# askerlee/segtran

Hardware: AMD Instinct MI355X
Metric: train-step images/sec (cfg2, re-associated op order) (higher is better)
Workload: dtype f32; 1 GPU; REFUGE fundus 2D, segtran eff-b4, translayers 3, layercompress 1,1,2,2, 512x512, bs 6/GPU; global_batch=6, per_gpu_batch=6, parallelism=dp1, step=fwd+BCE/Dice+bwd+allreduce+clip+BertAdam, op_order=re-associated, ranks=1

## Files before the change

include/segx.h:

```cpp
#ifndef SEGX_H
#define SEGX_H
#include <stdint.h>
#ifdef __cplusplus
extern "C" {
#endif

int segx_version(void);
int segx_last_error(char* buf, int buflen);

enum { SEGX_EPI_NONE = 0, SEGX_EPI_GELU = 1 ,
       SEGX_EPI_SWISH = 2 ,
       SEGX_EPI_RELU = 3  };
enum { SEGX_BIAS_NONE = 0, SEGX_BIAS_N = 1 , SEGX_BIAS_M = 2  };
enum { SEGX_ENGINE_F32 = 0, SEGX_ENGINE_BF16X6 = 1 };
enum { SEGX_ENGINE_SEL_DEFAULT = 0, SEGX_ENGINE_SEL_F32 = 1, SEGX_ENGINE_SEL_BF16X6 = 2 };
enum { SEGX_TILE_AUTO = 0, SEGX_TILE_128x128 = 1, SEGX_TILE_64x64 = 2, SEGX_TILE_128x32 = 3, SEGX_TILE_32x128 = 4, SEGX_TILE_64x128 = 5,
       SEGX_TILE_256x128 = 6, SEGX_TILE_WS128x128 = 7, SEGX_TILE_WS128x256 = 8, SEGX_TILE_WS64x256 = 9,
       SEGX_TILE_WS96x256 = 10, SEGX_TILE_WS256x96 = 11,
       SEGX_TILE_SKINNY_NT = 12   };
typedef struct {
    int32_t M, N, K, nb0, nb1;
    int64_t a_b0, a_b1, a_m, a_k;
    int64_t b_b0, b_b1, b_n, b_k;
    int64_t c_b0, c_b1, c_m;
    float alpha;
    int32_t epilogue, bias_mode;
    int64_t bias_b1;
    const float* bias;
    float* aux;
    float* gmax;
    float dropout_p;
    uint64_t seed, offset;
    int32_t splitk;
    float* workspace;
    int32_t tile;
    int64_t bias_b0;
    int32_t batch_reduce;
    int32_t engine;
    const void* b_planes;
    int64_t bp_b0, bp_b1;
    const float* resid;
} segx_gemm_desc;
int segx_gemm_f32(const float* A, const float* B, float* C, const segx_gemm_desc* d, void* stream);
int segx_gemm_plan(const float* A, const float* B, const segx_gemm_desc* d, int* tile, int* splitk);
int segx_gemm_plan_model(const float* A, const float* B, const segx_gemm_desc* d, int* tile, int* splitk);
int segx_gemm_route(const float* A, const float* B, const segx_gemm_desc* d, int32_t* out);
int64_t segx_x6_presplit_elems(int rows, int K, int nb0, int nb1);
int segx_x6_presplit(const float* W, int rows, int K, int64_t s_row, int64_t s_k, int nb0, int nb1, int64_t s_b0, int64_t s_b1, void* planes, void* stream);


int segx_softmax_fwd(const float* S, float* P, float* Pdrop, int64_t rows, int L, float clip, const float* gmax,
                     float p, uint64_t seed, uint64_t offset, void* stream);
int segx_softmax_bwd(const float* P, const float* dPdrop, const float* S , float* dS,
                     int64_t rows, int L, float clip, const float* gmax, float p, uint64_t seed, uint64_t offset, void* stream);
int segx_posbias_fwd(const float* S, float* out, const float* table, int64_t nmat, int N, const int* geom, float weight, float clip,
                     const float* gmax, void* stream);
int segx_posbias_bwd(const float* dOut, const float* S, float* dS, float* dtable, int64_t nmat, int N, const int* geom, float weight,
                     float clip, void* stream);
int segx_layernorm_fwd(const float* X, const float* w, const float* b, float* Y, float* mean, float* rstd,
                       int64_t rows, int C, float eps, void* stream);
int segx_layernorm_bwd(const float* dY, const float* X, const float* w, const float* mean, const float* rstd, float* dX,
                       int64_t rows, int C, void* stream);
int64_t segx_colreduce_ws_floats(int64_t rows, int64_t C, int nout);
int segx_colsum(const float* X, float* out, float* ws, int64_t rows, int64_t C, void* stream);
int segx_ln_param_grad(const float* dY, const float* X, const float* mean, const float* rstd, float* dw, float* db,
                       float* ws, int64_t rows, int C, void* stream);
int segx_sum(const float* x, int64_t n, float* out, float* ws , float scale, void* stream);
int segx_rowsum(const float* X, float* out, int64_t R, int64_t S, void* stream);
int segx_prenorm_fwd(const float* X, const float* w1, const float* b1, const float* pos, int64_t pos_ld, float pos_weight,
                     const float* mask, float* Y, float* stats, int64_t B, int N, int C, float eps,
                     float p, uint64_t seed, uint64_t offset, void* stream);
int segx_prenorm_bwd(const float* dY, const float* X, const float* w1, const float* b1, const float* pos, int64_t pos_ld,
                     float pos_weight, const float* mask, const float* stats, float* dX, float* dU, int64_t B, int N, int C,
                     float p, uint64_t seed, uint64_t offset, void* stream);
int64_t segx_prenorm_bwd_all_ws_floats(int N, int C);
int segx_prenorm_bwd_all(const float* dY, const float* X, const float* w1, const float* b1, const float* pos, int64_t pos_ld, float pos_weight,
                         const float* mask, const float* stats, float* dX, float* dsum, float* dw, float* db, float* ws, int B, int N, int C,
                         float p, uint64_t seed, uint64_t offset, void* stream);
int segx_posembed_fwd(const float* posn, const float* Wp, const float* bp, float* out, float* stats, int64_t N, int C, int pd,
                      float eps, void* stream);
int segx_posembed_bwd(const float* dOut, const float* posn, const float* Wp, const float* bp, const float* stats, float* dZ,
                      int64_t N, int C, int pd, void* stream);
int segx_modes_aggr_fwd(const float* Z, const float* lnw, const float* lnb, const float* wa, const float* ba, float* Y, float* stats,
                        int Mo, int64_t R, int F, float eps, float p, uint64_t seed, uint64_t offset, void* stream);
int segx_modes_aggr_bwd(const float* dY, const float* Z, const float* lnw, const float* lnb, const float* wa, const float* stats,
                        float* dZ, float* dscore, int Mo, int64_t R, int F, float p, uint64_t seed, uint64_t offset, void* stream);
int segx_modes_aggr_param_grad(const float* dY, const float* Z, const float* lnw, const float* lnb, const float* wa,
                               const float* stats, const float* dscore, float* dlnw, float* dlnb, float* dwa, float* ws,
                               int Mo, int64_t R, int F, float p, uint64_t seed, uint64_t offset, void* stream);
int64_t segx_modes_aggr_bwd_all_ws_floats(int Mo, int64_t R, int F);
int segx_modes_aggr_bwd_all(const float* dY, const float* Z, const float* lnw, const float* lnb, const float* wa, const float* stats,
                            float* dZ, float* dscore, float* dlnw, float* dlnb, float* dwa, float* ws, int Mo, int64_t R, int F,
                            float p, uint64_t seed, uint64_t offset, void* stream);
int segx_gelu_bwd(const float* dH, const float* T, float* dT, int64_t n, float p, uint64_t seed, uint64_t offset, void* stream);
int64_t segx_gelu_bwd_colsum_ws_floats(int64_t rows, int N);
int segx_gelu_bwd_colsum(const float* dH, const float* T, float* dT, float* colsum, float* ws, int64_t rows, int N, float p, uint64_t seed, uint64_t offset,
                         void* stream);

int64_t segx_loss_ws_floats(int B, int C);
int segx_seg_loss_fwd(const float* logits, const float* mask, const float* pos_weight, const float* class_w, float* out,
                      float* ws, int B, int C, int64_t S, float dice_w, void* stream);
// ... 221 lines not shown
```

segtran_amd/csrc/gemm.hip:

```cpp
#include "gemm_x6ws.h"
#include "gemm_skinny.h"
#include "gemm_tuned.h"

namespace segx {

template <class Cfg, bool AKC, bool BKC, bool VEC, int EPI>
__global__ __launch_bounds__(256, 2) void gemm_f32_kernel(GemmArgs g) {
    __shared__ __attribute__((aligned(16))) TileLdsT<Cfg> lds;
    const TileCoord t = tile_coord<Cfg>(g);
    const DenseLoader<AKC, VEC, Cfg::BM> la{g.A + t.z0 * g.a_b0 + t.z1 * g.a_b1, g.a_m, g.a_k, t.m0, g.M};
    const DenseLoader<BKC, VEC, Cfg::BN> lb{g.B + t.z0 * g.b_b0 + t.z1 * g.b_b1, g.b_n, g.b_k, t.n0, g.N};
    f32x16 acc[Cfg::MI][Cfg::NJ];
    gemm_mainloop<Cfg>(acc, la, lb, t.kbeg, t.kend, lds);
    gemm_epilogue<EPI, Cfg>(acc, g, t);
}

template <class Cfg, bool AKC, bool BKC, int EPI, int WPE, int VAR = 0, int TERMS = 6>
__global__ __launch_bounds__(256) SEGX_MIN_WAVES_PER_SIMD(WPE) void gemm_x6_kernel(GemmArgs g) {
    __shared__ __attribute__((aligned(16))) unsigned char lds[X6Lds<Cfg, TERMS>::BYTES];
    const TileCoord t = tile_coord<Cfg>(g);
    const DenseLoader6<AKC, Cfg::BM> la{g.A + t.z0 * g.a_b0 + t.z1 * g.a_b1, g.a_m, g.a_k, t.m0, g.M};
    const DenseLoader6<BKC, Cfg::BN> lb{g.B + t.z0 * g.b_b0 + t.z1 * g.b_b1, g.b_n, g.b_k, t.n0, g.N};
    f32x16 acc[Cfg::MI][Cfg::NJ];
    gemm_mainloop_x6<Cfg, DenseLoader6<AKC, Cfg::BM>, DenseLoader6<BKC, Cfg::BN>, VAR, TERMS>(acc, la, lb, t.kbeg, t.kend, lds);
// ... 370 lines not shown
static GemmLaunch ws3_kernel(const GemmRoute& r) {
    switch (r.tile) {
        case SEGX_TILE_256x128: return ws3_tile<Cfg256x128>(r);
        case SEGX_TILE_WS128x128: return ws3_tile<Cfg128>(r);
        case SEGX_TILE_WS128x256: return ws3_tile<Cfg128x256>(r);
        case SEGX_TILE_WS64x256: return built_for<Cfg64x256>(gemm_x6ws_kernel<Cfg64x256, true, false, SEGX_EPI_NONE, 0, 3>);
        case SEGX_TILE_WS96x256: return ws3_tile<Cfg96x256>(r);
        default: return built_for<Cfg256x96>(gemm_x6ws_kernel<Cfg256x96, true, true, SEGX_EPI_NONE, 0, 3>);
    }
}
template <class Cfg> static GemmLaunch ws_pre_tile(const GemmRoute& r) {
    return built_for<Cfg>(by_flag(r.akc, [](auto ak) -> GemmKernel { return gemm_x6ws_pre_kernel<Cfg, decltype(ak)::value>; }));
}
static GemmLaunch route_kernel(const GemmRoute& r) {
    if (r.terms == 3) {
        switch (r.family) {
            case GEMM_X6: return x3_kernel<false>(r);
#ifndef SEGX_NO_LEAN
            case GEMM_X6_LEAN: return x3_kernel<true>(r);
#endif
            default: return ws3_kernel(r);
        }
    }
    switch (r.family) {
        case GEMM_X6: return r.sched ? x6_sched_kernel(r.sched) : x6_kernel<false>(r);
#ifndef SEGX_NO_LEAN
        case GEMM_X6_LEAN: return x6_kernel<true>(r);
#endif
        case GEMM_WS: return ws_kernel(r);
        case GEMM_WS_PRE: return r.tile == SEGX_TILE_256x128 ? ws_pre_tile<Cfg256x128>(r) : ws_pre_tile<Cfg128x256>(r);
        default: return f32_kernel(r);
    }
}
static void set_tiles(GemmArgs& g, const GemmLaunch& k, const GemmRoute& r) {
    g.tiles_m = ceil_div(g.M, k.bm); g.tiles_n = ceil_div(g.N, k.bn); g.mfast = r.walk ? tile_walk(g.M, g.N, g.K, g.tiles_m) : 0;
}
static int persistent_grid(const GemmArgs& g, const GemmRoute& r, int* grid) {
    const int64_t items = (int64_t)g.tiles_m * g.tiles_n * g.nbatch * g.splitk;
    SEGX_REQUIRE(items < 2147483647LL - 512, "segx_gemm_f32: too many tiles");
    *grid = (int)i64min(r.ws_grid, (items + 7) / 8 * 8);
    return 0;
}
static void slab_reduce(const segx_gemm_desc* d, float* C, const float* bias, int nslabs, bool skinny, hipStream_t stream) {
    const int64_t total = (int64_t)d->M * d->N;
    const float* ws = static_cast<const float*>(d->workspace);
    if (total * 16 <= 512 * 1024 && nslabs >= 16)
        hipLaunchKernelGGL((slab_sum_parts_kernel<16>), dim3((unsigned)((total + 15) / 16)), dim3(256), 0, stream, ws, C, bias, d->M, d->N, nslabs, total, d->c_m, d->alpha, d->bias_mode);
    else if (skinny || (total * 4 <= 1024 * 1024 && nslabs >= 4))
        hipLaunchKernelGGL((slab_sum_parts_kernel<4>), dim3((unsigned)((total + 63) / 64)), dim3(256), 0, stream, ws, C, bias, d->M, d->N, nslabs, total, d->c_m, d->alpha, d->bias_mode);
    else
        SEGX_SPLITK_REDUCE((unsigned)i64min(2048, (total + 255) / 256), stream, ws, C, bias, d->M, d->N, 1, nslabs, total, (int64_t)0, (int64_t)0, d->c_m, d->alpha,
                           d->bias_mode, (int64_t)0, (int64_t)0, total, (const float*)nullptr);
}
}

extern "C" int segx_gemm_plan(const float* A, const float* B, const segx_gemm_desc* d, int* tile, int* splitk) { return segx::gemm_plan_impl(A, B, d, tile, splitk, true); }
extern "C" int segx_gemm_plan_model(const float* A, const float* B, const segx_gemm_desc* d, int* tile, int* splitk) { return segx::gemm_plan_impl(A, B, d, tile, splitk, false); }

extern "C" int segx_gemm_route(const float* A, const float* B, const segx_gemm_desc* d, int32_t* out) {
    using namespace segx;
    SEGX_REQUIRE(A && B && d && out && d->M > 0 && d->N > 0 && d->K > 0 && d->nb0 > 0 && d->nb1 > 0, "segx_gemm_route: bad args");
    SEGX_REQUIRE(d->tile >= SEGX_TILE_AUTO && d->tile <= SEGX_TILE_SKINNY_NT && d->engine >= SEGX_ENGINE_SEL_DEFAULT && d->engine <= SEGX_ENGINE_SEL_BF16X6,
                 "segx_gemm_route: bad tile %d or engine selector %d", d->tile, d->engine);
    GemmRoute r;
    const int rc = gemm_route(A, B, d, &r);
    if (rc) return rc;
    out[0] = r.family; out[1] = r.tile; out[2] = r.terms; out[3] = r.splitk;
    return 0;
}

extern "C" int segx_gemm_f32(const float* A, const float* B, float* C, const segx_gemm_desc* d, void* stream_) {
    using namespace segx;
    hipStream_t stream = (hipStream_t)stream_;
    SEGX_REQUIRE(A && B && C && d, "segx_gemm_f32: null pointer");
    SEGX_REQUIRE(d->M > 0 && d->N > 0 && d->K > 0 && d->nb0 > 0 && d->nb1 > 0, "segx_gemm_f32: bad sizes M=%d N=%d K=%d nb=%dx%d",
                 d->M, d->N, d->K, d->nb0, d->nb1);
    SEGX_REQUIRE(d->a_m == 1 || d->a_k == 1, "segx_gemm_f32: A needs a unit stride (a_m=%lld a_k=%lld)", (long long)d->a_m, (long long)d->a_k);
    SEGX_REQUIRE(d->b_n == 1 || d->b_k == 1, "segx_gemm_f32: B needs a unit stride (b_n=%lld b_k=%lld)", (long long)d->b_n, (long long)d->b_k);
    SEGX_REQUIRE(d->epilogue == SEGX_EPI_NONE || d->epilogue == SEGX_EPI_GELU || d->epilogue == SEGX_EPI_SWISH || d->epilogue == SEGX_EPI_RELU, "segx_gemm_f32: bad epilogue %d", d->epilogue);
    SEGX_REQUIRE(d->epilogue != SEGX_EPI_RELU || (d->a_k == 1 && d->b_n == 1 && d->b_k != 1 && !d->resid && !d->gmax && d->dropout_p == 0.f),
                 "segx_gemm_f32: the relu epilogue is built for a pointwise convolution's forward (A k-contiguous, B row-contiguous; no resid, gmax or dropout)");
    SEGX_REQUIRE(d->epilogue != SEGX_EPI_SWISH || (d->a_k == 1 && d->b_n == 1 && d->b_k != 1 && !d->resid && !d->gmax && d->dropout_p == 0.f),
                 "segx_gemm_f32: the swish epilogue is built for a pointwise convolution's forward (A k-contiguous, B row-contiguous; no resid, gmax or dropout)");
    SEGX_REQUIRE(d->epilogue != SEGX_EPI_GELU || d->aux, "segx_gemm_f32: GELU epilogue needs aux");
    SEGX_REQUIRE(d->bias_mode == SEGX_BIAS_NONE || d->bias, "segx_gemm_f32: bias_mode set but bias null");
    SEGX_REQUIRE(d->dropout_p >= 0.f && d->dropout_p < 1.f, "segx_gemm_f32: dropout_p out of range");
    const int splitk = d->splitk > 1 ? d->splitk : 1;
    SEGX_REQUIRE(splitk == 1 || (d->workspace && d->epilogue == SEGX_EPI_NONE && !d->gmax), "segx_gemm_f32: split-K needs workspace and a plain epilogue");
    const bool breduce = d->batch_reduce != 0;
    SEGX_REQUIRE(!breduce || (d->workspace && d->epilogue == SEGX_EPI_NONE && !d->gmax), "segx_gemm_f32: batch_reduce needs workspace and a plain epilogue");
    SEGX_REQUIRE(!d->resid || (d->epilogue == SEGX_EPI_NONE && !breduce && !d->gmax), "segx_gemm_f32: resid needs a plain epilogue (no GELU, no batch_reduce, no gmax)");
    SEGX_REQUIRE(d->tile >= SEGX_TILE_AUTO && d->tile <= SEGX_TILE_SKINNY_NT, "segx_gemm_f32: bad tile %d", d->tile);
    SEGX_REQUIRE(d->engine >= SEGX_ENGINE_SEL_DEFAULT && d->engine <= SEGX_ENGINE_SEL_BF16X6, "segx_gemm_f32: bad engine selector %d", d->engine);
    GemmRoute r;
    int rc = gemm_route(A, B, d, &r);
    if (rc) return rc;

    const int nbatch = d->nb0 * d->nb1;
    const float* bias = d->bias_mode ? d->bias : nullptr;
    if (r.family == GEMM_SKINNY) {
        const int nslabs = splitk * nbatch;
        rc = launch_skinny_nt(A, B, static_cast<float*>(d->workspace), d->M, d->N, d->K, d->nb0, d->nb1, d->a_b0, d->a_b1, d->a_m, d->b_b0, d->b_b1, d->b_n, nslabs, stream);
        if (rc) return rc;
        slab_reduce(d, C, bias, nslabs, true, stream);
        return check_launch("segx_gemm_f32/skinny_nt_reduce");
    }
// ... 63 lines not shown
```

segtran_amd/csrc/gemm_skinny.h:

```cpp
#pragma once
#include <cstdint>
#include <hip/hip_runtime.h>
namespace segx {
int skinny_nt_wgs_per_cu(int M, int N);
bool skinny_nt_shape_ok(int M, int N, int64_t K, int nbatch, int grid);
int launch_skinny_nt(const float* A, const float* B, float* ws, int M, int N, int64_t K, int nb0, int nb1, int64_t a_b0, int64_t a_b1, int64_t a_m,
                     int64_t b_b0, int64_t b_b1, int64_t b_n, int grid, hipStream_t stream);
}
```

segtran_amd/csrc/gemm_skinny.hip:

```cpp
#include "common.h"
#include "gemm_skinny.h"

namespace segx {

constexpr int SK_KT = 64, SK_LDW = SK_KT + 4, SK_T = 512;

struct SkinnyArgs {
    const float* A; const float* B; float* ws;
    int M, N, nb1, tpb;
    int64_t a_b0, a_b1, a_m, b_b0, b_b1, b_n;
    int64_t total;
};

template <int MB, int NB>
__global__ __launch_bounds__(SK_T) void gemm_skinny_nt_kernel(SkinnyArgs g) {
    constexpr int ROWS = (MB + NB) * 32, BUF = ROWS * SK_LDW;
    constexpr int NLD = (ROWS * 16 + SK_T - 1) / SK_T;
    __shared__ __attribute__((aligned(16))) float lds[2 * BUF];
    static_assert(2 * BUF * 4 <= 160 * 1024 && 8 * 1024 <= 2 * BUF, "LDS image");
    const int tid = threadIdx.x, lane = tid & 63, w = tid >> 6, r = lane & 31, h = lane >> 5;
    for (int i = tid; i < 2 * BUF / 4; i += SK_T) reinterpret_cast<f32x4*>(lds)[i] = f32x4{0.f, 0.f, 0.f, 0.f};
    const int nA = g.M * 16, nAll = (g.M + g.N) * 16;
    int goff[NLD], loff[NLD]; bool isA[NLD], valid[NLD];
#pragma unroll
    for (int i = 0; i < NLD; ++i) {
        const int f = tid + i * SK_T;
        valid[i] = f < nAll;
        isA[i] = !valid[i] || f < nA;
        const int row = !valid[i] ? 0 : (isA[i] ? f >> 4 : (f - nA) >> 4), c4 = f & 15;
        goff[i] = (int)((int64_t)row * (isA[i] ? g.a_m : g.b_n)) + (valid[i] ? c4 * 4 : 0);
        loff[i] = ((isA[i] ? row : MB * 32 + row) * SK_LDW + c4 * 4);
    }
    const int64_t t0 = g.total * blockIdx.x / gridDim.x, t1 = g.total * (blockIdx.x + 1) / gridDim.x;
    f32x16 acc[MB][NB];
#pragma unroll
    for (int i = 0; i < MB; ++i)
#pragma unroll
        for (int j = 0; j < NB; ++j)
#pragma unroll
            for (int q = 0; q < 16; ++q) acc[i][j][q] = 0.f;
    f32x4 pre[NLD];
    auto issue = [&](int64_t t) {
        const int64_t b = t / g.tpb; const int64_t k0 = (t - b * g.tpb) * SK_KT;
        const int64_t z0 = b / g.nb1, z1 = b - z0 * g.nb1;
        const float* pa = g.A + z0 * g.a_b0 + z1 * g.a_b1 + k0; const float* pb = g.B + z0 * g.b_b0 + z1 * g.b_b1 + k0;
#pragma unroll
        for (int i = 0; i < NLD; ++i) pre[i] = *reinterpret_cast<const f32x4*>((isA[i] ? pa : pb) + goff[i]);
    };
    auto stash = [&](int buf) {
#pragma unroll
        for (int i = 0; i < NLD; ++i) if (valid[i]) *reinterpret_cast<f32x4*>(lds + buf * BUF + loff[i]) = pre[i];
    };
    __syncthreads();
    if (t0 < t1) { issue(t0); stash(0); }
    __syncthreads();
    for (int64_t t = t0; t < t1; ++t) {
        const int cur = (int)((t - t0) & 1);
        const bool more = t + 1 < t1;
        if (more) issue(t + 1);
        const float* la = lds + cur * BUF + r * SK_LDW + 8 * w + 4 * h;
        f32x4 a[MB], bq[NB];
#pragma unroll
        for (int i = 0; i < MB; ++i) a[i] = *reinterpret_cast<const f32x4*>(la + i * 32 * SK_LDW);
#pragma unroll
        for (int j = 0; j < NB; ++j) bq[j] = *reinterpret_cast<const f32x4*>(la + (MB + j) * 32 * SK_LDW);
#pragma unroll
        for (int e = 0; e < 4; ++e)
#pragma unroll
            for (int i = 0; i < MB; ++i)
#pragma unroll
                for (int j = 0; j < NB; ++j) acc[i][j] = __builtin_amdgcn_mfma_f32_32x32x2f32(a[i][e], bq[j][e], acc[i][j], 0, 0, 0);
        if (more) stash(cur ^ 1);
        __syncthreads();
    }
    float* red = lds;
    float* slab = g.ws + (int64_t)blockIdx.x * g.M * g.N;
#pragma unroll
    for (int i = 0; i < MB; ++i)
#pragma unroll
        for (int j = 0; j < NB; ++j) {
#pragma unroll
            for (int q = 0; q < 16; ++q) red[w * 1024 + (8 * (q >> 2) + 4 * h + (q & 3)) * 32 + r] = acc[i][j][q];
            __syncthreads();
#pragma unroll
            for (int e = tid; e < 1024; e += SK_T) {
                float s = red[e];
#pragma unroll
                for (int v = 1; v < 8; ++v) s += red[v * 1024 + e];
                const int gm = i * 32 + (e >> 5), gn = j * 32 + (e & 31);
                if (gm < g.M && gn < g.N) slab[(int64_t)gm * g.N + gn] = s;
            }
            __syncthreads();
        }
}

int skinny_nt_wgs_per_cu(int M, int N) { const int rows = ((M + 31) / 32 + (N + 31) / 32) * 32; return rows <= 64 ? 3 : rows <= 96 ? 2 : 1; }

bool skinny_nt_shape_ok(int M, int N, int64_t K, int nbatch, int grid) {
    const int mb = (M + 31) / 32, nb = (N + 31) / 32;
    if (!(mb >= 1 && nb >= 1 && (mb == 1 || nb == 1) && mb <= 6 && nb <= 6)) return false;
    if (K % SK_KT != 0) return false;
    return (int64_t)nbatch * (K / SK_KT) >= 8LL * grid;
}

int launch_skinny_nt(const float* A, const float* B, float* ws, int M, int N, int64_t K, int nb0, int nb1, int64_t a_b0, int64_t a_b1, int64_t a_m,
                     int64_t b_b0, int64_t b_b1, int64_t b_n, int grid, hipStream_t stream) {
    SkinnyArgs g;
    g.A = A; g.B = B; g.ws = ws; g.M = M; g.N = N; g.nb1 = nb1; g.tpb = (int)(K / SK_KT);
    g.a_b0 = a_b0; g.a_b1 = a_b1; g.a_m = a_m; g.b_b0 = b_b0; g.b_b1 = b_b1; g.b_n = b_n;
    g.total = (int64_t)nb0 * nb1 * g.tpb;
    const int mb = (M + 31) / 32, nb = (N + 31) / 32;
#define SEGX_SKINNY(MB_, NB_) hipLaunchKernelGGL((gemm_skinny_nt_kernel<MB_, NB_>), dim3(grid), dim3(SK_T), 0, stream, g)
    if (nb == 1) switch (mb) { case 1: SEGX_SKINNY(1, 1); break; case 2: SEGX_SKINNY(2, 1); break; case 3: SEGX_SKINNY(3, 1); break;
                               case 4: SEGX_SKINNY(4, 1); break; case 5: SEGX_SKINNY(5, 1); break; default: SEGX_SKINNY(6, 1); break; }
    else switch (nb) { case 2: SEGX_SKINNY(1, 2); break; case 3: SEGX_SKINNY(1, 3); break; case 4: SEGX_SKINNY(1, 4); break;
                       case 5: SEGX_SKINNY(1, 5); break; default: SEGX_SKINNY(1, 6); break; }
#undef SEGX_SKINNY
    return check_launch("segx_gemm_f32/skinny_nt");
}

}
```

segtran_amd/functional.py:

```python
import math
import torch
import torch.nn.functional as F
from . import segx
from .segx import EPI_NONE, EPI_GELU, EPI_SWISH, EPI_RELU, BIAS_NONE, BIAS_N, BIAS_M

LN_EPS = 1e-12


_MRO = torch.autograd.Function.__mro__
_fast_apply = torch._C._FunctionBase in _MRO and not any('apply' in c.__dict__ for c in _MRO[1:_MRO.index(torch._C._FunctionBase)])


class _Fn(torch.autograd.Function):

    @classmethod
    def apply(cls, *args):
        if _fast_apply and not torch._C._are_functorch_transforms_active():
            return super(torch.autograd.Function, cls).apply(*args)
        return super().apply(*args)


def _live(t):
    return t.requires_grad and torch.is_grad_enabled()

# ... 62 lines not shown
        dc_as_rows = (s.c[0], s.c[1], s.c[2], 1) if which == 'a' else (s.c[0], s.c[1], 1, s.c[2])
        oth = (ost[0], ost[1], ost[3], ost[2])
        if k_contig:
            _run_gemm(L, dC, other, tmp, rows, cols, inner, dc_as_rows, oth, (tgt_b[0], tgt_b[1], row_stride), nb, s.alpha)
        else:
            _run_gemm(L, other, dC, tmp, cols, rows, inner, oth, dc_as_rows, (tgt_b[0], tgt_b[1], row_stride), nb, s.alpha)
        out = torch.empty_like(like)
        L.colsum(tmp, out, _empty(dC, L.colreduce_ws(nb[bd], n, 1)), nb[bd], n)
        return out
    if any(bcast) and like.is_contiguous() and like.numel() == rows * cols and (st[2] == 1 or st[3] == 1):
        k_contig = st[3] == 1
        out = torch.empty_like(like)
        dc_as_rows = (s.c[0], s.c[1], s.c[2], 1) if which == 'a' else (s.c[0], s.c[1], 1, s.c[2])
        oth = (ost[0], ost[1], ost[3], ost[2])
        if k_contig:
            _run_gemm(L, dC, other, out, rows, cols, inner, dc_as_rows, oth, (0, 0, cols), nb, s.alpha, batch_reduce=True)
        else:
            _run_gemm(L, other, dC, out, cols, rows, inner, oth, dc_as_rows, (0, 0, rows), nb, s.alpha, batch_reduce=True)
        return out
    if any(bcast):
        assert st[2] == 1 or st[3] == 1
        k_contig = st[3] == 1
        tmp_rows, tmp_cols = (rows, cols) if k_contig else (cols, rows)
        tmp = _empty(dC, nb[0] * nb[1], tmp_rows, tmp_cols)
        tb = (nb[1] * tmp_rows * tmp_cols, tmp_rows * tmp_cols)
        out_rs = tmp_cols
        tgt, tgt_b, row_stride = tmp, tb, out_rs
    else:
        k_contig = st[3] == 1
        tgt = torch.zeros_like(like) if not like.is_contiguous() else torch.empty_like(like)
        tgt_b, row_stride = (st[0], st[1]), (st[2] if k_contig else st[3])
    if which == 'a':
        dc_as_rows = (s.c[0], s.c[1], s.c[2], 1)
        oth = (ost[0], ost[1], ost[3], ost[2])
    else:
        dc_as_rows = (s.c[0], s.c[1], 1, s.c[2])
        oth = (ost[0], ost[1], ost[3], ost[2])
    kw = dict(resid=resid) if resid is not None else {}
    if k_contig:
        _run_gemm(L, dC, other, tgt, rows, cols, inner, dc_as_rows, oth, (tgt_b[0], tgt_b[1], row_stride), nb, s.alpha, **kw)
    else:
        _run_gemm(L, other, dC, tgt, cols, rows, inner, oth, dc_as_rows, (tgt_b[0], tgt_b[1], row_stride), nb, s.alpha, **kw)
    if any(bcast):
        assert all(bcast[i] or nb[i] == 1 for i in (0, 1)), 'partial batch broadcast is not supported'
        nbt = nb[0] * nb[1]
        out = torch.empty_like(like)
        assert like.is_contiguous() and like.numel() == tmp_rows * tmp_cols
        ws = _empty(dC, L.colreduce_ws(nbt, tmp_rows * tmp_cols, 1))
        L.colsum(tmp, out, ws, nbt, tmp_rows * tmp_cols)
        return out
    return tgt


class _BGemm(_Fn):
    gelu_bias_fused = True

    @staticmethod
    def forward(ctx, A, B, bias, spec, gmax, gelu, drop_p, pass_b=False):
        L = segx.lib()
        s = spec
        A, B = _c(A), _c(B)
        C = _empty(A, *s.out_shape)
        kw = dict(bias=bias, bias_mode=s.bias_mode if bias is not None else BIAS_NONE, bias_b1=s.bias_b1, bias_b0=s.bias_b0, gmax=gmax)
        T = None
        seed = off = 0
        if gelu:
            T = torch.empty_like(C)
            if drop_p > 0:
                seed, off = _Rng.reserve(C.numel())
            kw.update(epilogue=EPI_GELU, aux=T, dropout_p=drop_p, seed=seed, offset=off)
        _run_gemm(L, A, B, C, s.M, s.N, s.K, s.a, s.b, s.c, s.nb, s.alpha, **kw)
        ctx.spec, ctx.gelu, ctx.drop = s, gelu, (drop_p, seed, off)
        ctx.has_bias = bias is not None
        ctx.pass_b = pass_b
        ctx.set_materialize_grads(False)
        ctx.save_for_backward(A, B, T)
        if pass_b:
            return C, B.view_as(B)
        return C

    @staticmethod
    def backward(ctx, dC, dB_alias=None):
        L = segx.lib()
        A, B, T = ctx.saved_tensors
        s = ctx.spec
        if dC is None:
            return None, dB_alias, None, None, None, None, None, None
        dC = _c(dC)
        dbias = None
        if ctx.gelu:
            p, seed, off = ctx.drop
            dT = torch.empty_like(dC)
            if (ctx.has_bias and ctx.needs_input_grad[2] and s.bias_mode == BIAS_N and s.bias_b0 == 0 and (s.nb[1] == 1 or s.bias_b1 == 0) and s.c[2] == s.N
                    and s.N % 4 == 0 and s.N <= 2048 and _BGemm.gelu_bias_fused and off % 4 == 0 and dC.data_ptr() % 16 == 0 and T.data_ptr() % 16 == 0):
                rows = dC.numel() // s.N
                dbias = _empty(dC, s.N)
                L.gelu_bwd_colsum(dC, T, dT, dbias, _empty(dC, L.gelu_bwd_colsum_ws(rows, s.N)), rows, s.N, p, seed, off)
            else:
                L.gelu_bwd(dC, T, dT, dC.numel(), p, seed, off)
            dC = dT
        dA = _grad_operand(L, dC, B, s, 'a', A) if ctx.needs_input_grad[0] else None
        dB = _grad_operand(L, dC, A, s, 'b', B, resid=_c(dB_alias) if dB_alias is not None else None) if ctx.needs_input_grad[1] else None
        if dbias is None and ctx.has_bias and ctx.needs_input_grad[2]:
            dbias = _bias_grad(L, dC, s)
        return dA, dB, dbias, None, None, None, None, None


def _tag_plane_sums(dbase, rsum, B, C, S):
    dbase._segx_plane_sums = (rsum, dbase._version, dbase.data_ptr(), (int(B), int(C), int(S)))


def _take_plane_sums(dC, nbt, M, N):
    tag = getattr(dC, '_segx_plane_sums', None)
    if tag is None:
        return None
    del dC._segx_plane_sums
    rs, version, ptr, bcs = tag
    if version != dC._version or ptr != dC.data_ptr() or bcs != (int(nbt), int(M), int(N)) or not dC.is_contiguous() or rs.device != dC.device:
        return None
    return rs


def _bias_grad(L, dC, s):
    nb0, nb1 = s.nb
    assert s.c[2] == s.N or (s.bias_mode == BIAS_N and s.bias_b0 != 0), 'bias grad needs contiguous C rows'
    if s.bias_mode == BIAS_N and s.bias_b0 != 0:
        assert s.bias_b0 == nb1 * s.N and s.bias_b1 == s.N
        ones = torch.ones(s.M, dtype=torch.float32, device=dC.device)
        out = _empty(dC, nb0, nb1, s.N)
        _run_gemm(L, ones, dC, out, 1, s.N, s.M, (0, 0, s.M, 1), (s.c[0], s.c[1], 1, s.c[2]), (nb1 * s.N, s.N, s.N), s.nb, 1.0)
        return out
    if s.bias_mode == BIAS_N:
        if nb1 == 1 or s.bias_b1 == 0:
            rows = dC.numel() // s.N
            out = _empty(dC, s.N)
            L.colsum(dC, out, _empty(dC, L.colreduce_ws(rows, s.N, 1)), rows, s.N)
            return out
        assert nb0 == 1 and s.bias_b1 == s.N, 'grouped bias grad layout'
        out = _empty(dC, nb1 * s.N)
        for z in range(nb1):
            L.colsum(dC[z] if dC.dim() == 3 else dC.view(nb1, s.M, s.N)[z], out[z * s.N:(z + 1) * s.N],
                     _empty(dC, L.colreduce_ws(s.M, s.N, 1)), s.M, s.N)
        return out
    assert s.bias_b1 == 0
    nbt = nb0 * nb1
    rs = _take_plane_sums(dC, nbt, s.M, s.N)
    if rs is None:
        rs = _empty(dC, nbt * s.M)
        L.rowsum(dC, rs, nbt * s.M, s.N)
    if s.bias_b0 == s.M and nb1 == 1:
        return rs.view(nb0, s.M)
    if nbt == 1:
        return rs
    out = _empty(dC, s.M)
    L.colsum(rs, out, _empty(dC, L.colreduce_ws(nbt, s.M, 1)), nbt, s.M)
# ... 2265 lines not shown
```

segtran_amd/segx.py:

```python
import contextlib
import ctypes
import enum
import os
import torch

_HERE = os.path.dirname(os.path.abspath(__file__))
LIB_PATH = os.path.join(_HERE, 'lib', 'libsegx.so')

c_f = ctypes.c_float
c_i = ctypes.c_int32
c_l = ctypes.c_int64
c_u = ctypes.c_uint64
c_p = ctypes.c_void_p


class GemmDesc(ctypes.Structure):
    _fields_ = [('M', c_i), ('N', c_i), ('K', c_i), ('nb0', c_i), ('nb1', c_i),
                ('a_b0', c_l), ('a_b1', c_l), ('a_m', c_l), ('a_k', c_l),
                ('b_b0', c_l), ('b_b1', c_l), ('b_n', c_l), ('b_k', c_l),
                ('c_b0', c_l), ('c_b1', c_l), ('c_m', c_l),
                ('alpha', c_f), ('epilogue', c_i), ('bias_mode', c_i), ('bias_b1', c_l),
                ('bias', c_p), ('aux', c_p), ('gmax', c_p),
                ('dropout_p', c_f), ('seed', c_u), ('offset', c_u),
                ('splitk', c_i), ('workspace', c_p), ('tile', c_i), ('bias_b0', c_l), ('batch_reduce', c_i), ('engine', c_i),
# ... 146 lines not shown
        d.M, d.N, d.K, d.nb0, d.nb1 = M, N, K, nb[0], nb[1]
        d.a_b0, d.a_b1, d.a_m, d.a_k = a_strides
        d.b_b0, d.b_b1, d.b_n, d.b_k = b_strides
        d.c_b0, d.c_b1, d.c_m = c_strides
        d.alpha, d.epilogue, d.bias_mode, d.bias_b1, d.bias_b0 = alpha, epilogue, bias_mode, bias_b1, bias_b0
        d.bias, d.aux, d.gmax = _ptr(bias), _ptr(aux), _ptr(gmax)
        d.dropout_p, d.seed, d.offset = dropout_p, seed, offset
        if b_planes is not None:
            self._chk_t(b_planes[0])
            d.b_planes, d.bp_b0, d.bp_b1 = _ptr(b_planes[0]), b_planes[1], b_planes[2]
        d.engine = 0 if engine is None else 1 + self.ENGINES[engine]
        d.batch_reduce = 1 if batch_reduce else 0
        if splitk == 0:
            t, sk = c_i(0), c_i(0)
            self.check(self.c.segx_gemm_plan(_ptr(A), _ptr(B), ctypes.byref(d), ctypes.byref(t), ctypes.byref(sk)), 'segx_gemm_plan')
            tile, splitk = t.value, sk.value
            workspace = torch.empty(splitk * nb[0] * nb[1] * M * N, dtype=torch.float32, device=C.device) if (splitk > 1 or batch_reduce) else None
        d.splitk, d.workspace = splitk, _ptr(workspace)
        d.tile = self.force_tile if self.force_tile is not None else tile
        if self.gemm_prof is not None and C.is_cuda:
            e0, e1 = torch.cuda.Event(enable_timing=True), torch.cuda.Event(enable_timing=True)
            self.x6_launches()
            e0.record()
            rc = self.c.segx_gemm_f32(_ptr(A), _ptr(B), _ptr(C), ctypes.byref(d), self.stream(C))
            e1.record()
            self.gemm_prof.append((e0, e1, 2.0 * M * N * K * nb[0] * nb[1], (M, N, K, nb[0] * nb[1], a_strides[3] == 1, b_strides[3] == 1, splitk, d.tile),
                                   self.x6_launches() > 0))
        else:
            rc = self.c.segx_gemm_f32(_ptr(A), _ptr(B), _ptr(C), ctypes.byref(d), self.stream(C))
        self.check(rc, 'segx_gemm_f32')

    ROUTE_FAMILIES = ('f32', 'x6', 'x6_lean', 'ws', 'ws_pre', 'skinny')

    def gemm_route(self, A, B, M, N, K, a_strides, b_strides, nb=(1, 1), epilogue=EPI_NONE, splitk=1, tile=TILE_AUTO, engine=None):
        self._chk_t(A, B)
        d = GemmDesc()
        d.M, d.N, d.K, d.nb0, d.nb1 = M, N, K, nb[0], nb[1]
        d.a_b0, d.a_b1, d.a_m, d.a_k = a_strides
        d.b_b0, d.b_b1, d.b_n, d.b_k = b_strides
        d.epilogue, d.splitk, d.tile = epilogue, splitk, tile
        d.engine = 0 if engine is None else 1 + self.ENGINES[engine]
        out = (c_i * 4)()
        self.check(self.c.segx_gemm_route(_ptr(A), _ptr(B), ctypes.byref(d), out), 'segx_gemm_route')
        return self.ROUTE_FAMILIES[out[0]], out[1], out[2], out[3]

    def x6_presplit(self, W, rows, K, s_row, s_k, nb=(1, 1), s_b=(0, 0)):
        e0, e1 = (nb[0] if s_b[0] else 1), (nb[1] if s_b[1] else 1)
        planes = torch.empty(self.c.segx_x6_presplit_elems(rows, K, e0, e1), dtype=torch.int16, device=W.device)
        self._chk_t(W)
        self.check(self.c.segx_x6_presplit(_ptr(W), rows, K, s_row, s_k, e0, e1, s_b[0], s_b[1], _ptr(planes), self.stream(W)), 'segx_x6_presplit')
        per = 3 * rows * K
        return planes, (e1 * per if s_b[0] else 0), (per if s_b[1] else 0)

    def _call(self, name, ref, *args):
        conv = []
        dev = None
        hip = not self.emulated
        for a in args:
            if isinstance(a, torch.Tensor):
                if hip and not a.is_cuda:
                    raise RuntimeError('libsegx (HIP) called with a CPU tensor')
                if dev is None:
                    dev = a.device
                elif a.device != dev:
                    raise AssertionError('tensors on different devices')
                assert a.is_contiguous(), name + ': non-contiguous tensor'
                conv.append(a.data_ptr())
            else:
                conv.append(a)
        rc = getattr(self.c, name)(*conv, self.stream(ref))
        if rc:
            self.check(rc, name)

    def colreduce_ws(self, rows, C, nout):
        return int(self.c.segx_colreduce_ws_floats(rows, C, nout))

    def softmax_fwd(self, S, P, Pdrop, rows, L, clip, gmax, p, seed, offset):
        self._call('segx_softmax_fwd', S, S, P, Pdrop, rows, L, clip, gmax, p, seed, offset)

    def softmax_bwd(self, P, dPd, S, dS, rows, L, clip, gmax, p, seed, offset):
        self._call('segx_softmax_bwd', P, P, dPd, S, dS, rows, L, clip, gmax, p, seed, offset)

    def posbias_fwd(self, S, out, table, nmat, N, geom, weight, clip, gmax):
        self._chk_t(S, out, table, gmax)
        rc = self.c.segx_posbias_fwd(_ptr(S), _ptr(out), _ptr(table), nmat, N, self._geom(geom), weight, clip, _ptr(gmax), self.stream(out))
        self.check(rc, 'segx_posbias_fwd')

    def posbias_bwd(self, dOut, S, dS, dtable, nmat, N, geom, weight, clip):
        self._chk_t(dOut, S, dS, dtable)
        rc = self.c.segx_posbias_bwd(_ptr(dOut), _ptr(S), _ptr(dS), _ptr(dtable), nmat, N, self._geom(geom), weight, clip, self.stream(dtable))
        self.check(rc, 'segx_posbias_bwd')

    def layernorm_fwd(self, X, w, b, Y, mean, rstd, rows, C, eps):
        self._call('segx_layernorm_fwd', X, X, w, b, Y, mean, rstd, rows, C, eps)

    def layernorm_bwd(self, dY, X, w, mean, rstd, dX, rows, C):
        self._call('segx_layernorm_bwd', X, dY, X, w, mean, rstd, dX, rows, C)

    def colsum(self, X, out, ws, rows, C):
        self._call('segx_colsum', X, X, out, ws, rows, C)

    def ln_param_grad(self, dY, X, mean, rstd, dw, db, ws, rows, C):
        self._call('segx_ln_param_grad', X, dY, X, mean, rstd, dw, db, ws, rows, C)

    def rowsum(self, X, out, R, S):
        self._call('segx_rowsum', X, X, out, R, S)
# ... 455 lines not shown
        self._call('segx_conv3d_unpack_wgrad', dWp, dWp, dW, Cout, Cin, KV)

    def maxpool3d_fwd(self, X, Y, arg, planes, geom):
        self._chk_t(X, Y, arg)
        rc = self.c.segx_maxpool3d_fwd(_ptr(X), _ptr(Y), _ptr(arg), planes, self._geom(geom), self.stream(Y))
        self.check(rc, 'segx_maxpool3d_fwd')

    def maxpool3d_bwd(self, dY, arg, dX, planes, geom, addend=None):
        self._chk_t(dY, arg, dX, addend)
        assert addend is None or (addend.is_contiguous() and addend.shape == dX.shape)
        rc = self.c.segx_maxpool3d_bwd(_ptr(dY), _ptr(arg), _ptr(dX), planes, self._geom(geom), _ptr(addend), self.stream(dX))
        self.check(rc, 'segx_maxpool3d_bwd')

    def dropout(self, x, y, n, p, seed, offset):
        self._call('segx_dropout', x, x, y, n, float(p), seed, offset)

    def interp_bwd_axis(self, dout, din, outer, n_out, n_in, inner, src_scale=0.0):
        self._call('segx_interp_linear_bwd_axis', dout, dout, din, outer, n_out, n_in, inner, float(src_scale))

    def mt_bertadam_step(self, tabs, ntensors, nchunks, chunk, max_global, max_tensor, sched, b1, b2, eps, ws):
        t = tabs
        self._call('segx_mt_bertadam_step', ws, t['params'], t['grads'], t['m'], t['v'], t['sizes'], t['chunk_tensor'],
                   t['chunk_off'], t['chunk_first'], t['active'], t['lr'], t['wd'], ntensors, nchunks, chunk,
                   max_global, max_tensor, sched, b1, b2, eps, ws)


    def mt_gather(self, src_tab, tabs, chunk_begin, nchunks, chunk):
        self._call('segx_mt_gather', src_tab, src_tab, tabs['grads'], tabs['sizes'], tabs['chunk_tensor'], tabs['chunk_off'],
                   chunk_begin, nchunks, chunk)


_SIGS = {
    'segx_posbias_fwd': 'ppplipffpp', 'segx_posbias_bwd': 'pppplipffp',
    'segx_softmax_fwd': 'ppplifpfuup', 'segx_softmax_bwd': 'pppplifpfuup',
    'segx_layernorm_fwd': 'pppppplifp', 'segx_layernorm_bwd': 'pppppplip',
    'segx_colreduce_ws_floats': 'lli', 'segx_colsum': 'pppllp', 'segx_ln_param_grad': 'ppppppplip',
    'segx_sum': 'plppfp', 'segx_rowsum': 'ppllp',
    'segx_prenorm_fwd': 'pppplfpppliiffuup',
    'segx_prenorm_bwd': 'ppppplfppppliifuup',
    'segx_prenorm_bwd_all_ws_floats': 'ii', 'segx_prenorm_bwd_all': 'ppppplfpppppppiiifuup',
    'segx_posembed_fwd': 'pppppliifp', 'segx_posembed_bwd': 'ppppppliip',
    'segx_modes_aggr_fwd': 'pppppppiliffuup', 'segx_modes_aggr_bwd': 'ppppppppilifuup',
    'segx_modes_aggr_param_grad': 'pppppppppppilifuup', 'segx_gelu_bwd': 'ppplfuup',
    'segx_gelu_bwd_colsum': 'ppppplifuup', 'segx_gelu_bwd_colsum_ws_floats': 'li', 'segx_modes_aggr_bwd_all_ws_floats': 'ili', 'segx_modes_aggr_bwd_all': 'ppppppppppppilifuup',
    'segx_loss_ws_floats': 'ii', 'segx_seg_loss_fwd': 'ppppppiilfp', 'segx_seg_loss_bwd': 'pppppppiilfp',
    'segx_mt_bertadam_step': 'pppppppppppiiifffddfpp', 'segx_mt_gather': 'pppppiiip',
    'segx_gn_ws_floats': 'iii', 'segx_groupnorm_fwd': 'pppppppiiilfp', 'segx_groupnorm_bwd': 'pppppppppiiilpp',
    'segx_interp_gn_nparts': 'li', 'segx_interp_linear_fwd_axis2_gn': 'pppliiiilipip', 'segx_groupnorm_fwd_parts': 'ppipppppiiilfp',
    'segx_groupnorm_stats_parts': 'pippifp', 'segx_gn_fold_bwd': 'pppppppppiiilp', 'segx_bridge_mask': 'ppppiiiiiiiiip', 'segx_gn_fold_bwd_proj': 'ppippppppppiiilp',
    'segx_interp_linear_fwd': 'pppliiiiiip', 'segx_interp_linear_fwd_axis2': 'pppliiiilp', 'segx_interp_linear_bwd_axis2': 'ppliiiilp', 'segx_interp_linear_bwd': 'ppliiiiiip', 'segx_interp_linear_bwd_axis': 'ppliilfp',
    'segx_axis_gather': 'pplpp', 'segx_pixel_shuffle2': 'ppliiip', 'segx_add_noise': 'ppplffiuup', 'segx_resize2d': 'ppliiiiiip', 'segx_color_blend': 'ppilippip',
    'segx_gray_mean_ws_floats': 'il', 'segx_gray_mean': 'pppilip', 'segx_normalize': 'ppiilfppp',
    'segx_x6_presplit_elems': 'iiii', 'segx_x6_presplit': 'piilliillpp',
    'segx_tune': 'ii', 'segx_tune_get': 'i', 'segx_x3_launches': '', 'segx_gemm_route': 'pppp', 'segx_set_rng_base': 'p', 'segx_rng_advance': 'pup', 'segx_resized_crop3d': 'pplpp', 'segx_stem_compose_fwd': 'ppppiiiiip', 'segx_stem_compose_bwd': 'pppppppiiiiip', 'segx_bridge_input': 'ppiiiiiip', 'segx_stem_s2d_input': 'ppiiiiiip', 'segx_conv2d_stem_fwd': 'pppiiiiiiiiiiip', 'segx_conv2d_stem_im2col': 'ppiiiiiiiiiiip', 'segx_dropout': 'pplfuup', 'segx_avgpool2_fwd': 'ppliip', 'segx_avgpool2_bwd': 'ppliip', 'segx_transpose': 'ppliip', 'segx_interp_linear_fwd_axis': 'pppliilfp', 'segx_window_accum': 'pppiipp', 'segx_harden_segmap': 'ppppiilifp', 'segx_window_gather': 'ppppiiipp', 'segx_window_merge': 'pppppiiipifp', 'segx_dice_ws_floats': 'll', 'segx_dice_sums': 'pppllp',
    'segx_surface_border': 'ppliiiip', 'segx_edt_sq': 'ppliiip', 'segx_surface_hist': 'pppliiiip', 'segx_brats_case_tail': 'ppppplp',
    'segx_index_onehot': 'piplilp', 'segx_onehot_colormap': 'ppplilp', 'segx_onehot_case_tail': 'ppppppiilfp',
    'segx_ccl2d': 'pippliip', 'segx_frag_keep2': 'ppliip', 'segx_frag_apply': 'ppppliiip', 'segx_row_extent': 'ppliifp', 'segx_nhot_to_values': 'ppplilp',
    'segx_conv3d_fwd': 'pppiipipp', 'segx_conv3d_fwd_packed': 'pppiipipp', 'segx_conv3d_fwd_packed_bs': 'pppiipipllp', 'segx_conv3d_bwd_weight_packed_bs': 'pppiipipllp', 'segx_conv3d_pack_weights': 'ppiiiip', 'segx_conv3d_splitk': 'iipi', 'segx_conv3d_route': 'iipiiiip', 'segx_conv3d_fwd_terms': 'iipiii', 'segx_conv3d_flip_weights': 'ppiiip', 'segx_conv3d_bwd_weight': 'pppiipipp', 'segx_conv3d_bwd_weight_packed': 'pppiipipp', 'segx_conv3d_unpack_wgrad': 'ppiiip',
    'segx_conv3d_halo_ok': 'iip', 'segx_conv3d_halo_wq_floats': 'ii', 'segx_conv3d_halo_pack': 'ppiiip', 'segx_conv3d_halo_fwd': 'pppiipllip', 'segx_conv3d_halo_bias_act_fwd': 'ppppiiplliip', 'segx_conv3d_fwd_bias_act': 'ppppiipipillip', 'segx_bias_map_relu': 'ppilp', 'segx_conv3d_halo_wgrad_ok': 'iip', 'segx_conv3d_halo_wgrad_ws_floats': 'iip', 'segx_conv3d_halo_wgrad': 'ppppiipllp',
    'segx_conv3d_bwd_data_direct': 'ppppiipp', 'segx_nonzero_mask': 'ppiiiiiiiip', 'segx_label_nhot': 'ppiilip',
    'segx_maxpool3d_fwd': 'ppplpp', 'segx_maxpool3d_bwd': 'ppplppp',
    'segx_bn_ws_floats': 'iil', 
    'segx_dwconv2d_fwd': 'pppiiiiiiiiiip', 'segx_dwconv2d_bwd_data': 'pppiiiiiiiiiip',
    'segx_dwconv2d_pool_chunks': 'ii', 'segx_dwconv2d_bias_act_pool': 'pppppiiiiiiiiiiip', 'segx_conv2d_stem_bias_act_fwd': 'ppppiiiiiiiiiiiip',
    'segx_dwconv2d_bwd_weight': 'pppiiiiiiiiiip', 'segx_dwconv2d_bwd_weight_direct': 'pppiiiiiiiiiip', 'segx_dwconv2d_wgrad_rows': 'ii', 'segx_dwconv2d_bwd_fused_rows': 'iiiiiiii', 'segx_dwconv2d_bwd_fused': 'pppppiiiiiiiiiip', 'segx_plane_scale': 'pppllp', 'segx_plane_dot': 'pppllp',
     'segx_plane_bias_add': 'ppplilp',
    'segx_add_relu_fwd': 'pppplilp', 'segx_add_relu_bwd': 'pppllp',
    'segx_plane_chunks': 'l', 'segx_bn_pool_chunks': 'ili', 'segx_bn_parts_floats': 'iil', 'segx_bn_stats_local': 'pppiilp',
    'segx_bn_act_fwd2': 'ppippppfpppppfuuiilfillp', 'segx_bn_act_bwd2': 'ppppppppppiilfiippffuullp',
    'segx_team_status': 'i', 'segx_team_cap': '', 'segx_occupy': 'iifpp',
    'segx_mbconv_mid_ok': 'iiiii', 'segx_mbconv_mid_fwd': 'p' * 17 + 'ffff' + 'iiiii' + 'p', 'segx_mbconv_mid_bwd': 'p' * 19 + 'fff' + 'iiiii' + 'p',
    'segx_se_fwd2': 'pifpppppppppiiiip', 'segx_se_ws2_floats': 'iii', 'segx_se_bwd2': 'ppppppppfpppppppiiiip',
    'segx_bn_act_bwd_reduce': 'pppppppppiilfippffuup', 'segx_bn_act_bwd_apply': 'pppppppppiilfifppffuup',
}

_LIB = None
DEFAULT_ENGINE = 'x6'


def lib():
    global _LIB
    if _LIB is None:
        _LIB = SegxLib(LIB_PATH)
        _LIB.set_engine(os.environ.get('SEGX_ENGINE', DEFAULT_ENGINE))
    return _LIB


def use_library(libobj):
    global _LIB
    _LIB = libobj
```

Baseline: 99.00 images/s.

## Fuse 1x1-conv weight and input gradients into one streaming skinny kernel

Adds a pointwise-conv backward kernel for narrow input channel counts (at most 32) that streams dY and X tiles once. From the same LDS tiles it accumulates the weight gradient via the skinny NT MFMA path and computes dX = W^T·dY with 16x16x4 MFMAs using weights held in registers. The autograd backward of the batched GEMM routes eligible conv1x1 specs to this kernel instead of two separate GEMMs. This removes a second read of dY and one launch, at the cost of more LDS, more register pressure and extra per-iteration dX stores.

```diff
diff --git a/include/segx.h b/include/segx.h
--- a/include/segx.h
+++ b/include/segx.h
@@ -47,6 +47,9 @@
 int segx_gemm_route(const float* A, const float* B, const segx_gemm_desc* d, int32_t* out);
 int64_t segx_x6_presplit_elems(int rows, int K, int nb0, int nb1);
 int segx_x6_presplit(const float* W, int rows, int K, int64_t s_row, int64_t s_k, int nb0, int nb1, int64_t s_b0, int64_t s_b1, void* planes, void* stream);
+int segx_pwconv_bwd_narrow_ok(int B, int Cout, int Cin, int64_t S);
+int64_t segx_pwconv_bwd_narrow_ws_floats(int B, int Cout, int Cin, int64_t S);
+int segx_pwconv_bwd_narrow(const float* dY, const float* X, const float* W, float* dX, float* dW, float* ws, int B, int Cout, int Cin, int64_t S, void* stream);
 
 
 int segx_softmax_fwd(const float* S, float* P, float* Pdrop, int64_t rows, int L, float clip, const float* gmax,
diff --git a/segtran_amd/csrc/gemm.hip b/segtran_amd/csrc/gemm.hip
--- a/segtran_amd/csrc/gemm.hip
+++ b/segtran_amd/csrc/gemm.hip
@@ -446,6 +446,11 @@
         SEGX_SPLITK_REDUCE((unsigned)i64min(2048, (total + 255) / 256), stream, ws, C, bias, d->M, d->N, 1, nslabs, total, (int64_t)0, (int64_t)0, d->c_m, d->alpha,
                            d->bias_mode, (int64_t)0, (int64_t)0, total, (const float*)nullptr);
 }
+void skinny_slab_sum(const float* ws, float* C, int M, int N, int nslabs, hipStream_t stream) {
+    segx_gemm_desc d{};
+    d.M = M; d.N = N; d.c_m = N; d.alpha = 1.f; d.bias_mode = SEGX_BIAS_NONE; d.workspace = const_cast<float*>(ws);
+    slab_reduce(&d, C, nullptr, nslabs, true, stream);
+}
 }
 
 extern "C" int segx_gemm_plan(const float* A, const float* B, const segx_gemm_desc* d, int* tile, int* splitk) { return segx::gemm_plan_impl(A, B, d, tile, splitk, true); }
diff --git a/segtran_amd/csrc/gemm_skinny.h b/segtran_amd/csrc/gemm_skinny.h
--- a/segtran_amd/csrc/gemm_skinny.h
+++ b/segtran_amd/csrc/gemm_skinny.h
@@ -6,4 +6,5 @@
 bool skinny_nt_shape_ok(int M, int N, int64_t K, int nbatch, int grid);
 int launch_skinny_nt(const float* A, const float* B, float* ws, int M, int N, int64_t K, int nb0, int nb1, int64_t a_b0, int64_t a_b1, int64_t a_m,
                      int64_t b_b0, int64_t b_b1, int64_t b_n, int grid, hipStream_t stream);
+void skinny_slab_sum(const float* ws, float* C, int M, int N, int nslabs, hipStream_t stream);
 }
diff --git a/segtran_amd/csrc/gemm_skinny.hip b/segtran_amd/csrc/gemm_skinny.hip
--- a/segtran_amd/csrc/gemm_skinny.hip
+++ b/segtran_amd/csrc/gemm_skinny.hip
@@ -12,12 +12,16 @@
     int64_t total;
 };
 
-template <int MB, int NB>
-__global__ __launch_bounds__(SK_T) void gemm_skinny_nt_kernel(SkinnyArgs g) {
+struct PwBwdArgs : SkinnyArgs { const float* W; float* dX; };
+
+constexpr int SK_DXS = 32 * SK_LDW;
+
+template <int MB, int NB, bool DX, typename Args>
+__device__ __forceinline__ void skinny_stream(const Args& g, float* lds) {
     constexpr int ROWS = (MB + NB) * 32, BUF = ROWS * SK_LDW;
     constexpr int NLD = (ROWS * 16 + SK_T - 1) / SK_T;
-    __shared__ __attribute__((aligned(16))) float lds[2 * BUF];
-    static_assert(2 * BUF * 4 <= 160 * 1024 && 8 * 1024 <= 2 * BUF, "LDS image");
+    static_assert((2 * BUF + (DX ? 2 * SK_DXS : 0)) * 4 <= 160 * 1024 && 8 * 1024 <= 2 * BUF, "LDS image");
+    static_assert(!DX || NB == 1, "the fused dX half is built for <= 32 input channels");
     const int tid = threadIdx.x, lane = tid & 63, w = tid >> 6, r = lane & 31, h = lane >> 5;
     for (int i = tid; i < 2 * BUF / 4; i += SK_T) reinterpret_cast<f32x4*>(lds)[i] = f32x4{0.f, 0.f, 0.f, 0.f};
     const int nA = g.M * 16, nAll = (g.M + g.N) * 16;
@@ -51,9 +55,26 @@
 #pragma unroll
         for (int i = 0; i < NLD; ++i) if (valid[i]) *reinterpret_cast<f32x4*>(lds + buf * BUF + loff[i]) = pre[i];
     };
+    constexpr int NS = DX ? MB * 8 : 1;
+    const int pg = w >> 1, cih = w & 1, lq = lane >> 4, lj = lane & 15;
+    float wreg[NS];
+    bool dx_on = false;
+    int64_t xb = t0 / g.tpb; int xk = (int)(t0 - xb * g.tpb);
+    if constexpr (DX) {
+        dx_on = cih * 16 < g.N;
+#pragma unroll
+        for (int s = 0; s < NS; ++s) {
+            const int co = 16 * (s >> 2) + (s & 3) + 4 * lq, ci = cih * 16 + lj;
+            wreg[s] = (co < g.M && ci < g.N) ? g.W[(int64_t)co * g.N + ci] : 0.f;
+        }
+    }
     __syncthreads();
     if (t0 < t1) { issue(t0); stash(0); }
     __syncthreads();
+    if constexpr (DX) {
+#pragma unroll
+        for (int s = 0; s < NS; ++s) SEGX_PIN(wreg[s]);
+    }
     for (int64_t t = t0; t < t1; ++t) {
         const int cur = (int)((t - t0) & 1);
         const bool more = t + 1 < t1;
@@ -70,8 +91,29 @@
             for (int i = 0; i < MB; ++i)
 #pragma unroll
                 for (int j = 0; j < NB; ++j) acc[i][j] = __builtin_amdgcn_mfma_f32_32x32x2f32(a[i][e], bq[j][e], acc[i][j], 0, 0, 0);
+        if constexpr (DX) {
+            if (dx_on) {
+                const float* ly = lds + cur * BUF + 4 * lq * SK_LDW + 16 * pg + lj;
+                f32x4 d0 = {0.f, 0.f, 0.f, 0.f}, d1 = {0.f, 0.f, 0.f, 0.f};
+#pragma unroll
+                for (int s = 0; s < NS; s += 2) {
+                    d0 = __builtin_amdgcn_mfma_f32_16x16x4f32(wreg[s], ly[(16 * (s >> 2) + (s & 3)) * SK_LDW], d0, 0, 0, 0);
+                    d1 = __builtin_amdgcn_mfma_f32_16x16x4f32(wreg[s + 1], ly[(16 * ((s + 1) >> 2) + ((s + 1) & 3)) * SK_LDW], d1, 0, 0, 0);
+                }
+                float* st = lds + 2 * BUF + cur * SK_DXS + (16 * cih + 4 * lq) * SK_LDW + 16 * pg + lj;
+#pragma unroll
+                for (int q = 0; q < 4; ++q) st[q * SK_LDW] = d0[q] + d1[q];
+            }
+        }
         if (more) stash(cur ^ 1);
         __syncthreads();
+        if constexpr (DX) {
+            const int row = tid >> 4, c4 = tid & 15;
+            if (row < g.N)
+                *reinterpret_cast<f32x4*>(g.dX + xb * g.b_b0 + (int64_t)row * g.b_n + (int64_t)xk * SK_KT + c4 * 4) =
+                    *reinterpret_cast<const f32x4*>(lds + 2 * BUF + cur * SK_DXS + row * SK_LDW + c4 * 4);
+            if (++xk == g.tpb) { xk = 0; ++xb; }
+        }
     }
     float* red = lds;
     float* slab = g.ws + (int64_t)blockIdx.x * g.M * g.N;
@@ -92,6 +134,18 @@
             }
             __syncthreads();
         }
+}
+
+template <int MB, int NB>
+__global__ __launch_bounds__(SK_T) void gemm_skinny_nt_kernel(SkinnyArgs g) {
+    __shared__ __attribute__((aligned(16))) float lds[2 * (MB + NB) * 32 * SK_LDW];
+    skinny_stream<MB, NB, false>(g, lds);
+}
+
+template <int MB>
+__global__ __launch_bounds__(SK_T) void pwconv_bwd_narrow_kernel(PwBwdArgs g) {
+    __shared__ __attribute__((aligned(16))) float lds[2 * (MB + 1) * 32 * SK_LDW + 2 * SK_DXS];
+    skinny_stream<MB, 1, true>(g, lds);
 }
 
 int skinny_nt_wgs_per_cu(int M, int N) { const int rows = ((M + 31) / 32 + (N + 31) / 32) * 32; return rows <= 64 ? 3 : rows <= 96 ? 2 : 1; }
@@ -119,4 +173,40 @@
     return check_launch("segx_gemm_f32/skinny_nt");
 }
 
-}
+static int pwconv_bwd_narrow_grid(int B, int Cout, int Cin, int64_t S) {
+    if (!kget(knobs().skinny_nt) || B < 1 || Cout < 1 || Cin < 1 || Cin > 32 || Cout > 192 || S < SK_KT || S % SK_KT != 0) return 0;
+    if ((int64_t)Cout * S >= (1LL << 31)) return 0;
+    const int64_t total = (int64_t)B * (S / SK_KT), full = kget(knobs().ws_grid);
+    const int64_t grid = i64min(full, total / 8);
+    return grid >= 1 && 2 * grid >= full ? (int)grid : 0;
+}
+
+}
+
+extern "C" int segx_pwconv_bwd_narrow_ok(int B, int Cout, int Cin, int64_t S) { return segx::pwconv_bwd_narrow_grid(B, Cout, Cin, S) > 0 ? 1 : 0; }
+extern "C" int64_t segx_pwconv_bwd_narrow_ws_floats(int B, int Cout, int Cin, int64_t S) {
+    return (int64_t)segx::pwconv_bwd_narrow_grid(B, Cout, Cin, S) * Cout * Cin;
+}
+extern "C" int segx_pwconv_bwd_narrow(const float* dY, const float* X, const float* W, float* dX, float* dW, float* ws, int B, int Cout, int Cin, int64_t S,
+                                      void* stream_) {
+    using namespace segx;
+    hipStream_t stream = (hipStream_t)stream_;
+    const int grid = pwconv_bwd_narrow_grid(B, Cout, Cin, S);
+    SEGX_REQUIRE(grid > 0, "segx_pwconv_bwd_narrow: B=%d Cout=%d Cin=%d S=%lld is not a shape of this kernel (segx_pwconv_bwd_narrow_ok)", B, Cout, Cin, (long long)S);
+    SEGX_REQUIRE(dY && X && W && dX && dW && ws, "segx_pwconv_bwd_narrow: null pointer");
+    SEGX_REQUIRE(((reinterpret_cast<uintptr_t>(dY) | reinterpret_cast<uintptr_t>(X) | reinterpret_cast<uintptr_t>(dX) | reinterpret_cast<uintptr_t>(ws)) & 15) == 0,
+                 "segx_pwconv_bwd_narrow: 16-byte alignment");
+    PwBwdArgs g;
+    g.A = dY; g.B = X; g.ws = ws; g.M = Cout; g.N = Cin; g.nb1 = 1; g.tpb = (int)(S / SK_KT);
+    g.a_b0 = (int64_t)Cout * S; g.a_b1 = 0; g.a_m = S; g.b_b0 = (int64_t)Cin * S; g.b_b1 = 0; g.b_n = S;
+    g.total = (int64_t)B * g.tpb;
+    g.W = W; g.dX = dX;
+#define SEGX_PWBWD(MB_) hipLaunchKernelGGL((pwconv_bwd_narrow_kernel<MB_>), dim3(grid), dim3(SK_T), 0, stream, g)
+    switch ((Cout + 31) / 32) { case 1: SEGX_PWBWD(1); break; case 2: SEGX_PWBWD(2); break; case 3: SEGX_PWBWD(3); break;
+                                case 4: SEGX_PWBWD(4); break; case 5: SEGX_PWBWD(5); break; default: SEGX_PWBWD(6); break; }
+#undef SEGX_PWBWD
+    int rc = check_launch("segx_pwconv_bwd_narrow");
+    if (rc) return rc;
+    skinny_slab_sum(ws, dW, Cout, Cin, grid, stream);
+    return check_launch("segx_pwconv_bwd_narrow/reduce");
+}
diff --git a/segtran_amd/functional.py b/segtran_amd/functional.py
--- a/segtran_amd/functional.py
+++ b/segtran_amd/functional.py
@@ -138,7 +138,12 @@
     return tgt
 
 
+def _is_conv1x1_spec(s):
+    return (s.nb[1] == 1 and s.a == (0, 0, s.K, 1) and s.b == (s.K * s.N, 0, 1, s.N) and s.c == (s.M * s.N, 0, s.N) and s.alpha == 1.0)
+
+
 class _BGemm(_Fn):
+    fused_narrow_backward = True
     gelu_bias_fused = True
 
     @staticmethod
@@ -158,6 +163,7 @@
         _run_gemm(L, A, B, C, s.M, s.N, s.K, s.a, s.b, s.c, s.nb, s.alpha, **kw)
         ctx.spec, ctx.gelu, ctx.drop = s, gelu, (drop_p, seed, off)
         ctx.has_bias = bias is not None
+        ctx.has_gmax = gmax is not None
         ctx.pass_b = pass_b
         ctx.set_materialize_grads(False)
         ctx.save_for_backward(A, B, T)
@@ -185,8 +191,13 @@
             else:
                 L.gelu_bwd(dC, T, dT, dC.numel(), p, seed, off)
             dC = dT
-        dA = _grad_operand(L, dC, B, s, 'a', A) if ctx.needs_input_grad[0] else None
-        dB = _grad_operand(L, dC, A, s, 'b', B, resid=_c(dB_alias) if dB_alias is not None else None) if ctx.needs_input_grad[1] else None
+        if (_BGemm.fused_narrow_backward and ctx.needs_input_grad[0] and ctx.needs_input_grad[1] and not ctx.gelu and not ctx.has_gmax and dB_alias is None
+                and _is_conv1x1_spec(s) and not (dC.data_ptr() | A.data_ptr() | B.data_ptr()) % 16 and L.pwconv_bwd_narrow_ok(s.nb[0], s.M, s.K, s.N)):
+            dA, dB = torch.empty_like(A), torch.empty_like(B)
+            L.pwconv_bwd_narrow(dC, B, A, dB, dA, s.nb[0], s.M, s.K, s.N)
+        else:
+            dA = _grad_operand(L, dC, B, s, 'a', A) if ctx.needs_input_grad[0] else None
+            dB = _grad_operand(L, dC, A, s, 'b', B, resid=_c(dB_alias) if dB_alias is not None else None) if ctx.needs_input_grad[1] else None
         if dbias is None and ctx.has_bias and ctx.needs_input_grad[2]:
             dbias = _bias_grad(L, dC, s)
         return dA, dB, dbias, None, None, None, None, None
diff --git a/segtran_amd/segx.py b/segtran_amd/segx.py
--- a/segtran_amd/segx.py
+++ b/segtran_amd/segx.py
@@ -222,6 +222,13 @@
         per = 3 * rows * K
         return planes, (e1 * per if s_b[0] else 0), (per if s_b[1] else 0)
 
+    def pwconv_bwd_narrow_ok(self, B, Cout, Cin, S):
+        return bool(self.c.segx_pwconv_bwd_narrow_ok(B, Cout, Cin, S))
+
+    def pwconv_bwd_narrow(self, dY, X, W, dX, dW, B, Cout, Cin, S):
+        ws = torch.empty(int(self.c.segx_pwconv_bwd_narrow_ws_floats(B, Cout, Cin, S)), dtype=torch.float32, device=dY.device)
+        self._call('segx_pwconv_bwd_narrow', dY, dY, X, W, dX, dW, ws, B, Cout, Cin, S)
+
     def _call(self, name, ref, *args):
         conv = []
         dev = None
@@ -783,6 +790,7 @@
     'segx_axis_gather': 'pplpp', 'segx_pixel_shuffle2': 'ppliiip', 'segx_add_noise': 'ppplffiuup', 'segx_resize2d': 'ppliiiiiip', 'segx_color_blend': 'ppilippip',
     'segx_gray_mean_ws_floats': 'il', 'segx_gray_mean': 'pppilip', 'segx_normalize': 'ppiilfppp',
     'segx_x6_presplit_elems': 'iiii', 'segx_x6_presplit': 'piilliillpp',
+    'segx_pwconv_bwd_narrow_ok': 'iiil', 'segx_pwconv_bwd_narrow_ws_floats': 'iiil', 'segx_pwconv_bwd_narrow': 'ppppppiiilp',
     'segx_tune': 'ii', 'segx_tune_get': 'i', 'segx_x3_launches': '', 'segx_gemm_route': 'pppp', 'segx_set_rng_base': 'p', 'segx_rng_advance': 'pup', 'segx_resized_crop3d': 'pplpp', 'segx_stem_compose_fwd': 'ppppiiiiip', 'segx_stem_compose_bwd': 'pppppppiiiiip', 'segx_bridge_input': 'ppiiiiiip', 'segx_stem_s2d_input': 'ppiiiiiip', 'segx_conv2d_stem_fwd': 'pppiiiiiiiiiiip', 'segx_conv2d_stem_im2col': 'ppiiiiiiiiiiip', 'segx_dropout': 'pplfuup', 'segx_avgpool2_fwd': 'ppliip', 'segx_avgpool2_bwd': 'ppliip', 'segx_transpose': 'ppliip', 'segx_interp_linear_fwd_axis': 'pppliilfp', 'segx_window_accum': 'pppiipp', 'segx_harden_segmap': 'ppppiilifp', 'segx_window_gather': 'ppppiiipp', 'segx_window_merge': 'pppppiiipifp', 'segx_dice_ws_floats': 'll', 'segx_dice_sums': 'pppllp',
     'segx_surface_border': 'ppliiiip', 'segx_edt_sq': 'ppliiip', 'segx_surface_hist': 'pppliiiip', 'segx_brats_case_tail': 'ppppplp',
     'segx_index_onehot': 'piplilp', 'segx_onehot_colormap': 'ppplilp', 'segx_onehot_case_tail': 'ppppppiilfp',
```

Result: no change. 99.67 images/s (median of 6 runs) (+0.7%).
